# Byshx/Poccala

Measured on AMD Instinct MI355X. Metric: frames/sec GMM-score+fwd-bwd, 39-d MFCC, 2048-mix, higher is better.
Workload: dtype f32-class (f16x2 split operands, f32 accumulate; f64 dynamic programming)

## Files before the change

### poccala_amd/csrc/gmm_score_split.hip

```cpp
#include <stdlib.h>

#include "pcl_internal.h"

namespace {

#ifndef PCL_SPLIT_WG
#define PCL_SPLIT_WG 256
#endif
constexpr int WG = PCL_SPLIT_WG;
typedef float f16v __attribute__((ext_vector_type(16)));

#ifndef PCL_SPLIT16_NT
#define PCL_SPLIT16_NT 2
#endif
#ifndef PCL_SPLIT16_MINW
#define PCL_SPLIT16_MINW 3
#endif
#ifndef PCL_SPLIT16_RING
#define PCL_SPLIT16_RING 2
#endif
#ifndef PCL_SPLIT16_MTS
#define PCL_SPLIT16_MTS 2
#endif
typedef _Float16 h8v __attribute__((ext_vector_type(8)));

template <int D>
struct Ring {
    static constexpr int KS8 = (D + 7) / 8;
    static constexpr int R = KS8 > 5 ? 2 : PCL_SPLIT16_RING;
    static constexpr int MTS = KS8 > 5 ? 1 : PCL_SPLIT16_MTS;
    static constexpr int STAGE_CH = MTS * 2 * KS8;
    static constexpr size_t LDS = (size_t)R * STAGE_CH * 64 * 16 + 16;
    static_assert(R >= 2 && MTS >= 1, "a ring has at least two stages");
    static_assert(3 * LDS <= (160u << 10), "three workgroups per CU: the ring does not fit a third of the 160 KB of LDS");
    static_assert(LDS <= (56u << 10), "pcl_score_occupancy(ctx, 2) pads a workgroup to 56 KB");
};

template <int N>
__device__ __forceinline__ void wait_vmcnt() {
    static_assert(N >= 0 && N < 64, "vmcnt is a 6-bit counter");
    asm volatile("s_waitcnt vmcnt(%0)" ::"n"(N) : "memory");
}

template <int D, int NT>
__global__ __launch_bounds__(WG, PCL_SPLIT16_MINW * 256 / WG > 0 ? PCL_SPLIT16_MINW * 256 / WG : 1) void gmm_score_split16_kernel(
    const float *__restrict__ frames, const uint4 *__restrict__ pm, const float *__restrict__ fscale, const float *__restrict__ centers,
    int nmt_max, const ScoreTile *__restrict__ tiles, const ScoreSeg *__restrict__ segs, double *__restrict__ out,
    int *__restrict__ flags, const double *__restrict__ kzero, const int *__restrict__ n_on_pipe, const int *__restrict__ npt) {
    static_assert(D % 8 != 0, "the folded constants need a spare slot");
    constexpr int KS8 = (D + 7) / 8;
    constexpr int CH = 2 * KS8;
    constexpr int SC = D / 8, JC = D % 8;
    constexpr float FMAXH = 6.0e4f;
    const ScoreTile tile = tiles[blockIdx.x];
    const int lane = threadIdx.x & 63;
    const int wave = threadIdx.x >> 6;
    const int half = lane >> 5;
    const int col = lane & 31;
    if (tile.seg_lo >= tile.seg_hi) {
        if (threadIdx.x == 0) flags[blockIdx.x] = 0;
        return;
    }
    const int n_mtiles = npt[tile.state];
    __shared__ int s_ovf;
    if (threadIdx.x == 0) s_ovf = 0;
    __syncthreads();
    const int vend = segs[tile.seg_hi - 1].vstart + segs[tile.seg_hi - 1].len;
    const bool wave_active = tile.vstart + wave * NT * 32 < vend;
    if (n_mtiles == 0) {
        if (wave_active) {
            for (int c = 0; c < NT; ++c) {
                const int v = tile.vstart + (wave * NT + c) * 32 + col;
                if (v < vend && half == 0) {
                    int lo = tile.seg0;
                    const int hi = tile.seg_hi - 1;
                    while (lo < hi && segs[lo + 1].vstart <= v) ++lo;
                    const ScoreSeg sg = segs[lo];
                    out[sg.out0 + (long long)(v - sg.vstart) * sg.out_stride] = -INFINITY;
                }
            }
        }
        if (threadIdx.x == 0) flags[blockIdx.x] = 0;
        return;
    }

    h8v xb[NT][2][KS8];
    long long oidx[NT];
    bool valid[NT];
    const float *cen = centers + (size_t)tile.state * D;
    const float *fs = fscale + ((size_t)tile.state * 2 + half) * (KS8 * 8);
    bool ovf = false;
#pragma unroll
    for (int c = 0; c < NT; ++c) {
        int v = tile.vstart + (wave * NT + c) * 32 + col;
        valid[c] = v < vend;
        if (!valid[c]) v = tile.vstart;
        int lo = tile.seg0, hi = tile.seg_hi - 1;
        if (lo < hi && segs[lo + 1].vstart <= v) {
            ++lo;
            if (lo < hi && segs[lo + 1].vstart <= v) {
                ++lo;
                while (lo < hi) {
                    int mid = (lo + hi + 1) >> 1;
                    if (segs[mid].vstart <= v) lo = mid; else hi = mid - 1;
                }
            }
        }
        const ScoreSeg sg = segs[lo];
        const long long t = v - sg.vstart;
        const float *fp = frames + (sg.frame0 + t) * D;
#pragma unroll
        for (int s = 0; s < KS8; ++s)
#pragma unroll
            for (int j = 0; j < 8; ++j) {
                const int d = 8 * s + j;
                float val = 0.f;
                if (d < D) {
                    const float xc = fp[d] - cen[d];
                    val = (half ? xc : xc * xc) * fs[d];
                    ovf |= __builtin_fabsf(val) > FMAXH;
                    val = __builtin_fminf(__builtin_fmaxf(val, -FMAXH), FMAXH);
                }
                if (d == D) val = half ? 0.f : 1.f;
                const _Float16 h1 = (_Float16)val;
                xb[c][0][s][j] = h1;
                xb[c][1][s][j] = (_Float16)(val - (float)h1);
            }
        oidx[c] = sg.out0 + t * (long long)sg.out_stride;
    }
    if (__any(ovf) && lane == 0) s_ovf = 1;

    float sm[NT], ref[NT];
    bool inited[NT];
#pragma unroll
    for (int c = 0; c < NT; ++c) {
        sm[c] = 0.f;
        ref[c] = 0.f;
        inited[c] = false;
    }
    bool ref_ovf = false;

    constexpr int R = Ring<D>::R, MTS = Ring<D>::MTS;
    __shared__ __attribute__((aligned(16))) uint4 abuf[R][MTS * CH * 64];
    const uint4 *pstate = pm + (size_t)tile.state * nmt_max * (CH * 64);
    const int wave_s = __builtin_amdgcn_readfirstlane(wave);
    auto dma = [&](int buf, int stage) {
        const uint4 *src = pstate + (size_t)stage * (MTS * CH * 64);
        const int nch = min(MTS, n_mtiles - stage * MTS) * CH;
        if constexpr (KS8 > 5) {
            for (int p = wave; p < nch; p += WG / 64)
                __builtin_amdgcn_global_load_lds((const __attribute__((address_space(1))) void *)(src + p * 64 + lane),
                                                 (__attribute__((address_space(3))) void *)&abuf[buf][p * 64], 16, 0, 0);
            return;
        }
#pragma unroll
        for (int i = 0; i < (MTS * CH + WG / 64 - 1) / (WG / 64); ++i) {
            const int p = wave_s + i * (WG / 64);
            if (p >= nch) continue;
            if constexpr (R == 2) {
                __builtin_amdgcn_global_load_lds((const __attribute__((address_space(1))) void *)(src + p * 64 + lane),
                                                 (__attribute__((address_space(3))) void *)&abuf[buf][p * 64], 16, 0, 0);
            } else {
                const unsigned lds = (unsigned)(size_t)(__attribute__((address_space(3))) char *)&abuf[buf][p * 64];
                asm volatile("s_mov_b32 m0, %0\n\ts_nop 0\n\tglobal_load_lds_dwordx4 %1, off"
                             :: "s"(lds), "v"(src + p * 64 + lane) : "memory");
            }
        }
    };

#ifdef PCL_SPLIT_STAMPS
    unsigned long long st_acc[4] = {0, 0, 0, 0}, st_t = 0;
#define SSTAMP(k) { const unsigned long long t_ = __builtin_amdgcn_s_memtime(); st_acc[k] += t_ - st_t; st_t = t_; }
#else
#define SSTAMP(k)
#endif
    auto process = [&](int mt) {
        const uint4 *ab = &abuf[(unsigned)(mt / MTS) % R][(mt % MTS) * (CH * 64)];
        f16v acc[NT];
#pragma unroll
        for (int c = 0; c < NT; ++c)
#pragma unroll
            for (int r = 0; r < 16; ++r) acc[c][r] = 0.f;
        auto frag = [&](int pa, int s) { return *reinterpret_cast<const h8v *>(&ab[(pa * KS8 + s) * 64 + lane]); };
        auto mfma = [&](const h8v &a, int c, int pb, int s) { acc[c] = __builtin_amdgcn_mfma_f32_32x32x16_f16(a, xb[c][pb][s], acc[c], 0, 0, 0); };
        float es[8], eh, snew[NT];
        auto lse_op = [&](int c, int k) {
            if (k < 24) {
                const int r = k / 3;
                if (k % 3 == 0) es[r] = __builtin_amdgcn_exp2f(acc[c][r]);
                else if (k % 3 == 1) eh = __builtin_amdgcn_exp2f(acc[c][r + 8]);
                else es[r] += eh;
            } else if (k < 28) es[k - 24] += es[k - 24 + 4];
            else if (k < 30) es[k - 28] += es[k - 28 + 2];
            else if (k == 30) es[0] += es[1];
            else snew[c] = sm[c] + es[0];
        };
        if constexpr (KS8 <= 5) {
            h8v af[2 * KS8];
            auto rd = [&](int f) { af[f] = frag(f < KS8 ? 1 : 0, f % KS8); };
            constexpr int LATE = KS8 > 2 ? 2 : 0;
            rd(0);
            rd(1);
            __builtin_amdgcn_sched_barrier(0);
#ifdef PCL_SPLIT_PRIO
            __builtin_amdgcn_s_setprio(1);
#endif
#pragma unroll
            for (int s = 0; s < KS8; ++s) {
#pragma unroll
                for (int c = 0; c < NT; ++c) {
                    mfma(af[s], c, 0, s);
                    if (s == 0 && c == 0) {
                        __builtin_amdgcn_sched_barrier(0);
#pragma unroll
                        for (int f = 2; f < 2 * KS8 - LATE; ++f) rd(f);
                    }
                }
                if (s == 2) {
#pragma unroll
                    for (int f = 2 * KS8 - LATE; f < 2 * KS8; ++f) rd(f);
                }
                __builtin_amdgcn_sched_barrier(0);
            }
#pragma unroll
            for (int c = 0; c < NT; ++c) {
                int k = 0;
#pragma unroll
                for (int g = 0; g < 2 * KS8; ++g) {
                    mfma(af[KS8 + g % KS8], c, g < KS8 ? 1 : 0, g % KS8);
                    if (c == 0) __builtin_amdgcn_sched_barrier(0);
#ifndef PCL_DIAG_NOLSE
                    if (c > 0) {
#pragma unroll
                        for (int q = 0; q < 3 && k < 32; ++q, ++k) lse_op(c - 1, k);
                        __builtin_amdgcn_sched_barrier(0);
                    }
#endif
                }
#ifndef PCL_DIAG_NOLSE
                if (c > 0) {
#pragma unroll
                    for (; k < 32; ++k) lse_op(c - 1, k);
                }
#endif
                __builtin_amdgcn_sched_barrier(0);
            }
        } else {
            auto pass = [&](int pa, int pb) {
#pragma unroll
                for (int s = 0; s < KS8; ++s) {
                    const h8v a = frag(pa, s);
#pragma unroll
                    for (int c = 0; c < NT; ++c) mfma(a, c, pb, s);
                }
            };
            pass(1, 0);
            pass(0, 1);
            pass(0, 0);
#ifndef PCL_DIAG_NOLSE
#pragma unroll
            for (int c = 0; c + 1 < NT; ++c)
#pragma unroll
                for (int k = 0; k < 32; ++k) lse_op(c, k);
#endif
        }
#ifndef PCL_DIAG_NOLSE
#pragma unroll
        for (int k = 0; k < 32; ++k) lse_op(NT - 1, k);
#endif
        SSTAMP(1)
#ifdef PCL_SPLIT_PRIO
        __builtin_amdgcn_s_setprio(0);
#endif
#ifdef PCL_DIAG_NOLSE
#pragma unroll
        for (int c = 0; c < NT; ++c) sm[c] += acc[c][0] + acc[c][15];
        return;
#endif
#pragma unroll
        for (int c = 0; c < NT; ++c) {
            if (__any(!inited[c]) | __any(!(snew[c] < 3.0e38f))) {
                float gm = acc[c][0];
#pragma unroll
                for (int r = 1; r < 16; ++r) gm = __builtin_fmaxf(gm, acc[c][r]);
                const float gp = __builtin_fmaxf(gm, __shfl_xor(gm, 32, 64));
                float s = sm[c];
                const bool first = !inited[c];
                if ((first || gp > 0.f) && gp > -5.0e4f) {
                    const _Float16 r1 = (_Float16)__builtin_fminf(__builtin_fmaxf(-(ref[c] + gp), -FMAXH), FMAXH);
                    const float nref = -(float)r1, dl = nref - ref[c];
                    ref_ovf |= __builtin_fabsf(nref) > 5.0e4f;
#ifdef PCL_LSE_FLUSH_REPRO
                    s = first ? 0.f : s * __builtin_amdgcn_exp2f(-dl);
#else
                    const float hs = __builtin_amdgcn_exp2f(-0.5f * dl);
                    s = first ? 0.f : (s * hs) * hs;
#endif
                    inited[c] = true;
#pragma unroll
                    for (int r = 0; r < 16; ++r) acc[c][r] -= dl;
                    ref[c] = nref;
                    if (half) xb[c][0][SC][JC] = r1;
                }
#pragma unroll
                for (int r = 0; r < 16; ++r) s += __builtin_amdgcn_exp2f(acc[c][r]);
                sm[c] = s;
            } else {
                sm[c] = snew[c];
            }
        }
        SSTAMP(2)
    };
    const int n_stages = (n_mtiles + MTS - 1) / MTS;
    dma(0, 0);
#pragma unroll
    for (int s = 1; s < R - 1; ++s)
        if (s < n_stages) dma(s, s);
#ifdef PCL_SPLIT_STAMPS
    st_t = __builtin_amdgcn_s_memtime();
#endif
    constexpr int NW = WG / 64, YLO = (R - 2) * ((MTS * CH) / NW), YHI = (R - 2) * ((MTS * CH) / NW + 1);
    for (int st = 0; st < n_stages; ++st) {
        if (R > 2 && (st + R - 1) * MTS <= n_mtiles) {
            if (wave_s < (MTS * CH) % NW) wait_vmcnt<YHI>(); else wait_vmcnt<YLO>();
        } else {
            wait_vmcnt<0>();
        }
        SSTAMP(3)
        if constexpr (R == 2) {
            __syncthreads();
        } else {
            asm volatile("s_waitcnt lgkmcnt(0)" ::: "memory");
            __builtin_amdgcn_s_barrier();
            asm volatile("" ::: "memory");
        }
        SSTAMP(0)
        if (st == 0 && threadIdx.x == 0) flags[blockIdx.x] = s_ovf;
        if (st + R - 1 < n_stages) dma((unsigned)(st + R - 1) % R, st + R - 1);
        if (wave_active) {
            const int mend = min(n_mtiles, (st + 1) * MTS);
            for (int mt = st * MTS; mt < mend; ++mt) process(mt);
        }
    }
#ifdef PCL_SPLIT_STAMPS
    if (blockIdx.x == 800 && lane == 0)
        printf("wave %d: per m-tile: dma-wait %llu  barrier %llu  dma-issue+lds+mfma %llu  lse %llu (memtime ticks)\n", wave,
               st_acc[3] / n_mtiles, st_acc[0] / n_mtiles, st_acc[1] / n_mtiles, st_acc[2] / n_mtiles);
#endif
    constexpr double LN2 = 0.693147180559945309417232121458;
    const double k0 = kzero[tile.state];
    if (wave_active && n_on_pipe[tile.state] > 0) {
#pragma unroll
        for (int c = 0; c < NT; ++c) ref_ovf |= !inited[c];
    }
#pragma unroll
    for (int c = 0; c < NT; ++c) {
        const double S = (double)sm[c] + (double)__shfl_xor(sm[c], 32, 64);
        if (valid[c] && half == 0) out[oidx[c]] = (S > 0) ? LN2 * ((double)ref[c] + k0 + ::log2(S)) : -INFINITY;
    }
    if (__any(ref_ovf) && lane == 0) s_ovf = 1;
    __syncthreads();
    if (threadIdx.x == 0 && s_ovf) flags[blockIdx.x] = 1;
}

template <int D>
void launch16_t(pcl_ctx *ctx, pcl_batch *b, const ScoreTile *tiles, int n_tiles) {
    constexpr size_t static_lds = Ring<D>::LDS;
    const size_t pad = (ctx->score_wgs_per_cu == 2 && static_lds < (56u << 10)) ? (56u << 10) - static_lds : 0;
    hipLaunchKernelGGL((gmm_score_split16_kernel<D, PCL_SPLIT16_NT>), dim3(n_tiles), dim3(WG), pad, ctx->stream, ctx->frames32,
                       reinterpret_cast<const uint4 *>(ctx->pm16f.p), ctx->fscale, ctx->centers32, ctx->Mpad32 / 32, tiles, b->d_segs,
                       b->Bt, b->d_tile_flags, ctx->kzero, ctx->d_non, ctx->d_npt);
}

}

int pcl_score_split16_tile_frames() { return WG / 64 * PCL_SPLIT16_NT * 32; }

int pcl_launch_score_split16(pcl_ctx *ctx, pcl_batch *b, const ScoreTile *tiles, int n_tiles) {
    if (n_tiles == 0) return PCL_OK;
    pcl_timer_begin(ctx, "score");
    switch (ctx->D) {
#define CASE(DD) case DD: launch16_t<DD>(ctx, b, tiles, n_tiles); break;
        PCL_MFMA_DIMS(CASE)
#undef CASE
        default: PCL_FAIL(ctx, PCL_ERR_INVALID, "internal: no split-f16 scoring kernel for D=%d", ctx->D);
    }
    pcl_timer_end(ctx, "score");
    HIPCHK(ctx, hipGetLastError());
    return PCL_OK;
}
```

Baseline: 22.45 million.

## Software-pipeline MFMA with carried log-sum-exp across column tiles in split16 kernel

Adds a carry path for the split16 GMM scoring kernel. The log-sum-exp of one column tile's accumulator is interleaved with the MFMA chain of the other tile, carried over from the previous m-tile, so exp2/add latency hides under matrix work, and a tail step drains the last carried accumulator. Output indices are stashed in LDS to free VGPRs, and lane/wave ids are recomputed via readfirstlane and mbcnt. This adds LDS, a fixed static LSE walk table and manual sched_barriers, and it changes reduction order slightly.

```diff
diff --git a/poccala_amd/csrc/gmm_score_split.hip b/poccala_amd/csrc/gmm_score_split.hip
--- a/poccala_amd/csrc/gmm_score_split.hip
+++ b/poccala_amd/csrc/gmm_score_split.hip
@@ -21,6 +21,9 @@
 #endif
 #ifndef PCL_SPLIT16_MTS
 #define PCL_SPLIT16_MTS 2
+#endif
+#ifndef PCL_SPLIT16_CARRY
+#define PCL_SPLIT16_CARRY 1
 #endif
 typedef _Float16 h8v __attribute__((ext_vector_type(8)));
 
@@ -30,7 +33,13 @@
     static constexpr int R = KS8 > 5 ? 2 : PCL_SPLIT16_RING;
     static constexpr int MTS = KS8 > 5 ? 1 : PCL_SPLIT16_MTS;
     static constexpr int STAGE_CH = MTS * 2 * KS8;
-    static constexpr size_t LDS = (size_t)R * STAGE_CH * 64 * 16 + 16;
+#ifdef PCL_DIAG_NOLSE
+    static constexpr bool CARRY = false;
+#else
+    static constexpr bool CARRY = PCL_SPLIT16_CARRY && KS8 <= 5 && PCL_SPLIT16_NT == 2;
+#endif
+    static constexpr size_t STASH = CARRY ? (size_t)WG * PCL_SPLIT16_NT * sizeof(long long) : 0;
+    static constexpr size_t LDS = (size_t)R * STAGE_CH * 64 * 16 + 16 + STASH;
     static_assert(R >= 2 && MTS >= 1, "a ring has at least two stages");
     static_assert(3 * LDS <= (160u << 10), "three workgroups per CU: the ring does not fit a third of the 160 KB of LDS");
     static_assert(LDS <= (56u << 10), "pcl_score_occupancy(ctx, 2) pads a workgroup to 56 KB");
@@ -67,10 +76,13 @@
     __syncthreads();
     const int vend = segs[tile.seg_hi - 1].vstart + segs[tile.seg_hi - 1].len;
     const bool wave_active = tile.vstart + wave * NT * 32 < vend;
+    const int wave_u = Ring<D>::CARRY ? __builtin_amdgcn_readfirstlane(wave) : 0;
     if (n_mtiles == 0) {
         if (wave_active) {
             for (int c = 0; c < NT; ++c) {
-                const int v = tile.vstart + (wave * NT + c) * 32 + col;
+                int v = tile.vstart + (wave * NT + c) * 32 + col;
+                if constexpr (Ring<D>::CARRY)
+                    v = tile.vstart + (wave_u * NT + c) * 32 + ((int)__builtin_amdgcn_mbcnt_hi(~0u, __builtin_amdgcn_mbcnt_lo(~0u, 0u)) & 31);
                 if (v < vend && half == 0) {
                     int lo = tile.seg0;
                     const int hi = tile.seg_hi - 1;
@@ -141,9 +153,15 @@
     bool ref_ovf = false;
 
     constexpr int R = Ring<D>::R, MTS = Ring<D>::MTS;
+    constexpr bool CARRY = Ring<D>::CARRY && NT == PCL_SPLIT16_NT;
     __shared__ __attribute__((aligned(16))) uint4 abuf[R][MTS * CH * 64];
     const uint4 *pstate = pm + (size_t)tile.state * nmt_max * (CH * 64);
     const int wave_s = __builtin_amdgcn_readfirstlane(wave);
+    __shared__ long long s_oidx[Ring<D>::CARRY ? NT : 1][Ring<D>::CARRY ? WG : 1];
+    if constexpr (Ring<D>::CARRY) {
+#pragma unroll
+        for (int c = 0; c < NT; ++c) s_oidx[c][wave_s * 64 + lane] = valid[c] ? oidx[c] : -1;
+    }
     auto dma = [&](int buf, int stage) {
         const uint4 *src = pstate + (size_t)stage * (MTS * CH * 64);
         const int nch = min(MTS, n_mtiles - stage * MTS) * CH;
@@ -174,6 +192,49 @@
 #else
 #define SSTAMP(k)
 #endif
+    auto lse_step = [&](const f16v &a, float (&t)[5], float &sn, int c, int k) {
+        constexpr signed char LSE_WALK[32][3] = {
+            {0, 0, 0}, {0, 1, 8},  {1, 0, 1}, {0, 1, 4}, {0, 2, 12}, {1, 1, 2}, {1, 0, 1},
+            {0, 1, 2}, {0, 2, 10}, {1, 1, 2}, {0, 2, 6}, {0, 3, 14}, {1, 2, 3}, {1, 1, 2}, {1, 0, 1},
+            {0, 1, 1}, {0, 2, 9},  {1, 1, 2}, {0, 2, 5}, {0, 3, 13}, {1, 2, 3}, {1, 1, 2},
+            {0, 2, 3}, {0, 3, 11}, {1, 2, 3}, {0, 3, 7}, {0, 4, 15}, {1, 3, 4}, {1, 2, 3}, {1, 1, 2},
+            {1, 0, 1}, {2, 0, 0}};
+        const int kind = LSE_WALK[k][0], dst = LSE_WALK[k][1], src = LSE_WALK[k][2];
+        if (kind == 0) t[dst] = __builtin_amdgcn_exp2f(a[src]);
+        else if (kind == 1) t[dst] += t[src];
+        else sn = sm[c] + t[0];
+    };
+    auto settle = [&](f16v &a, int c, float sn) {
+        if (__any(!inited[c]) | __any(!(sn < 3.0e38f))) {
+            float gm = a[0];
+#pragma unroll
+            for (int r = 1; r < 16; ++r) gm = __builtin_fmaxf(gm, a[r]);
+            const float gp = __builtin_fmaxf(gm, __shfl_xor(gm, 32, 64));
+            float s = sm[c];
+            const bool first = !inited[c];
+            if ((first || gp > 0.f) && gp > -5.0e4f) {
+                const _Float16 r1 = (_Float16)__builtin_fminf(__builtin_fmaxf(-(ref[c] + gp), -FMAXH), FMAXH);
+                const float nref = -(float)r1, dl = nref - ref[c];
+                ref_ovf |= __builtin_fabsf(nref) > 5.0e4f;
+#ifdef PCL_LSE_FLUSH_REPRO
+                s = first ? 0.f : s * __builtin_amdgcn_exp2f(-dl);
+#else
+                const float hs = __builtin_amdgcn_exp2f(-0.5f * dl);
+                s = first ? 0.f : (s * hs) * hs;
+#endif
+                inited[c] = true;
+#pragma unroll
+                for (int r = 0; r < 16; ++r) a[r] -= dl;
+                ref[c] = nref;
+                if (half) xb[c][0][SC][JC] = r1;
+            }
+#pragma unroll
+            for (int r = 0; r < 16; ++r) s += __builtin_amdgcn_exp2f(a[r]);
+            sm[c] = s;
+        } else {
+            sm[c] = sn;
+        }
+    };
     auto process = [&](int mt) {
         const uint4 *ab = &abuf[(unsigned)(mt / MTS) % R][(mt % MTS) * (CH * 64)];
         f16v acc[NT];
@@ -311,6 +372,67 @@
         }
         SSTAMP(2)
     };
+    f16v cacc[2];
+    if constexpr (CARRY) {
+#pragma unroll
+        for (int r = 0; r < 16; ++r) cacc[1][r] = -FMAXH;
+    }
+    auto process_carry = [&](int mt) {
+        const uint4 *ab = &abuf[(unsigned)(mt / MTS) % R][(mt % MTS) * (CH * 64)];
+        auto frag = [&](int pa, int s) { return *reinterpret_cast<const h8v *>(&ab[(pa * KS8 + s) * 64 + lane]); };
+        h8v af[2 * KS8];
+        auto rd = [&](int f) { af[f] = frag(f < KS8 ? 1 : 0, f % KS8); };
+        float t[5], snew;
+        rd(0);
+        rd(1);
+        __builtin_amdgcn_sched_barrier(0);
+#pragma unroll
+        for (int c = 0; c < 2; ++c) {
+            int k = 0;
+#pragma unroll
+            for (int g = 0; g < 3 * KS8; ++g) {
+                const int s = g % KS8;
+                const h8v &a = af[g < KS8 ? s : KS8 + s];
+                const h8v &x = xb[c][g >= KS8 && g < 2 * KS8 ? 1 : 0][s];
+                if (g == 0) {
+                    f16v zero;
+#pragma unroll
+                    for (int r = 0; r < 16; ++r) zero[r] = 0.f;
+                    cacc[c] = __builtin_amdgcn_mfma_f32_32x32x16_f16(a, x, zero, 0, 0, 0);
+                } else {
+                    cacc[c] = __builtin_amdgcn_mfma_f32_32x32x16_f16(a, x, cacc[c], 0, 0, 0);
+                }
+                if (g == 0) {
+                    __builtin_amdgcn_sched_barrier(0);
+                    if (c == 0) {
+#pragma unroll
+                        for (int f = 2; f < 2 * KS8; ++f) rd(f);
+                    }
+                }
+                if (c == 1 || g > 0) {
+#pragma unroll
+                    for (int q = 0; q < 3 && k < 32; ++q, ++k) lse_step(cacc[1 - c], t, snew, 1 - c, k);
+                }
+                __builtin_amdgcn_sched_barrier(0);
+            }
+#pragma unroll
+            for (; k < 32; ++k) lse_step(cacc[1 - c], t, snew, 1 - c, k);
+            __builtin_amdgcn_sched_barrier(0);
+            if (c == 0) {
+                settle(cacc[1], 1, snew);
+            } else {
+                SSTAMP(1)
+                settle(cacc[0], 0, snew);
+                SSTAMP(2)
+            }
+        }
+    };
+    auto carry_tail = [&]() {
+        float t[5], snew;
+#pragma unroll
+        for (int k = 0; k < 32; ++k) lse_step(cacc[1], t, snew, 1, k);
+        settle(cacc[1], 1, snew);
+    };
     const int n_stages = (n_mtiles + MTS - 1) / MTS;
     dma(0, 0);
 #pragma unroll
@@ -339,8 +461,13 @@
         if (st + R - 1 < n_stages) dma((unsigned)(st + R - 1) % R, st + R - 1);
         if (wave_active) {
             const int mend = min(n_mtiles, (st + 1) * MTS);
-            for (int mt = st * MTS; mt < mend; ++mt) process(mt);
-        }
+            for (int mt = st * MTS; mt < mend; ++mt) {
+                if constexpr (CARRY) process_carry(mt); else process(mt);
+            }
+        }
+    }
+    if constexpr (CARRY) {
+        if (wave_active) carry_tail();
     }
 #ifdef PCL_SPLIT_STAMPS
     if (blockIdx.x == 800 && lane == 0)
@@ -356,6 +483,10 @@
 #pragma unroll
     for (int c = 0; c < NT; ++c) {
         const double S = (double)sm[c] + (double)__shfl_xor(sm[c], 32, 64);
+        if constexpr (Ring<D>::CARRY) {
+            oidx[c] = s_oidx[c][wave_s * 64 + (int)__builtin_amdgcn_mbcnt_hi(~0u, __builtin_amdgcn_mbcnt_lo(~0u, 0u))];
+            valid[c] = oidx[c] >= 0;
+        }
         if (valid[c] && half == 0) out[oidx[c]] = (S > 0) ? LN2 * ((double)ref[c] + k0 + ::log2(S)) : -INFINITY;
     }
     if (__any(ref_ovf) && lane == 0) s_ovf = 1;
```

Result: faster. 22.76 million, median of 6 (+1.4%).
